# Vill-Lab/2023-TIFS-ISTVT

Hardware: AMD Instinct MI355X
Metric: clips/sec (BxTx3x224x224 fwd+bwd) (higher is better)
Workload: dtype bf16; 1 GPU; C2: B=32/GPU T=8 224x224 full ISTVT (Xception stem + 12-layer DSTTr) train step (fwd+bwd+grad all-reduce+SGD), random-init weights; global_batch=32, frames=8, size=224, depth=12, parallelism=dp1, early_allreduce=False, attn_fp8=False, dead_row_elimination=False, final_norm_class_rows_only=False, optimizer=SGD(momentum 0.9) fused, step_graphs=False

## Files before the change

### 2023-tifs-istvt_amd/csrc/attn_spatial.hip

```cpp
#include "common.h"
#include <type_traits>
#include <cstdlib>

constexpr int CHUNK = 128;
constexpr int NT = CHUNK / 16;
#ifdef ISTVT_SATTN_NOSTORE
#define SB_STORE4(p, v) do { if (scale < -1e30f) store4(p, v); } while (0)
#else
#define SB_STORE4(p, v) store4(p, v)
#endif
template <typename T, int DH> struct Pitch { static constexpr int v = DH + (sizeof(T) == 2 ? 16 : 8); };
#define LOG2E 1.4426950408889634f
#define LN2 0.6931471805599453f

template <typename T, int DH, int NTHR = 256>
__device__ __forceinline__ void stage_img(T* img, const T* __restrict__ src, long ld, int row0, int nrows, int tid) {
    constexpr int LDI = Pitch<T, DH>::v;
    constexpr int VPR = DH / 8;
    constexpr int NV = CHUNK * VPR / NTHR;
#pragma unroll
    for (int i = 0; i < NV; ++i) {
        const int v = tid + NTHR * i;
        const int row = v / VPR, col = (v % VPR) * 8;
        typename Mma<T>::frag f;
        if (row0 + row < nrows) f = frag_load(src + (long)(row0 + row) * ld + col);
        else f = Mma<T>::zero();
        if constexpr (sizeof(T) == 2) {
            *reinterpret_cast<bf16x8*>(img + row * LDI + col) = f;
        } else {
            float* p = (float*)(img + row * LDI + col);
            *reinterpret_cast<float4*>(p) = make_float4(f.v[0], f.v[1], f.v[2], f.v[3]);
            *reinterpret_cast<float4*>(p + 4) = make_float4(f.v[4], f.v[5], f.v[6], f.v[7]);
        }
    }
}

template <typename T, int DH, int NTHR>
struct StageRegs { typename Mma<T>::frag f[CHUNK * (DH / 8) / NTHR]; };
template <typename T, int DH, int NTHR>
__device__ __forceinline__ void stage_fetch(StageRegs<T, DH, NTHR>& rg, const T* __restrict__ src, long ld, int row0,
                                            int nrows, int tid) {
    constexpr int VPR = DH / 8;
    constexpr int NV = CHUNK * VPR / NTHR;
#pragma unroll
    for (int i = 0; i < NV; ++i) {
        const int v = tid + NTHR * i;
        const int row = v / VPR, col = (v % VPR) * 8;
        if (row0 + row < nrows) rg.f[i] = frag_load(src + (long)(row0 + row) * ld + col);
        else rg.f[i] = Mma<T>::zero();
    }
}
template <typename T, int DH, int NTHR>
__device__ __forceinline__ void stage_commit(T* img, const StageRegs<T, DH, NTHR>& rg, int tid, int rlim = CHUNK) {
    constexpr int LDI = Pitch<T, DH>::v;
    constexpr int VPR = DH / 8;
    constexpr int NV = CHUNK * VPR / NTHR;
#pragma unroll
    for (int i = 0; i < NV; ++i) {
        const int v = tid + NTHR * i;
        const int row = v / VPR, col = (v % VPR) * 8;
        if (row >= rlim) continue;
        if constexpr (sizeof(T) == 2) {
            *reinterpret_cast<bf16x8*>(img + row * LDI + col) = rg.f[i];
        } else {
            float* p = (float*)(img + row * LDI + col);
            *reinterpret_cast<float4*>(p) = make_float4(rg.f[i].v[0], rg.f[i].v[1], rg.f[i].v[2], rg.f[i].v[3]);
            *reinterpret_cast<float4*>(p + 4) = make_float4(rg.f[i].v[4], rg.f[i].v[5], rg.f[i].v[6], rg.f[i].v[7]);
        }
    }
}

template <typename T, int DH, int NTHR, int NCH>
__device__ __forceinline__ void stage_all2(T* imgA, const T* __restrict__ srcA, long ldA, T* imgB, const T* __restrict__ srcB,
                                           long ldB, int P, int tid, int img_rows) {
    constexpr int LDI = Pitch<T, DH>::v;
    StageRegs<T, DH, NTHR> ra[NCH], rb[NCH];
#pragma unroll
    for (int ch = 0; ch < NCH; ++ch) {
        if (ch * CHUNK < P) {
            stage_fetch(ra[ch], srcA, ldA, ch * CHUNK, P, tid);
            stage_fetch(rb[ch], srcB, ldB, ch * CHUNK, P, tid);
        }
    }
#pragma unroll
    for (int ch = 0; ch < NCH; ++ch) {
        if (ch * CHUNK < P) {
            stage_commit(imgA + ch * CHUNK * LDI, ra[ch], tid, img_rows - ch * CHUNK);
            stage_commit(imgB + ch * CHUNK * LDI, rb[ch], tid, img_rows - ch * CHUNK);
        }
    }
}

template <typename T>
__device__ __forceinline__ typename Mma<T>::frag row_frag(const T* __restrict__ src, long ld, int row, int nrows,
                                                           int col) {
    if (row < nrows) return frag_load(src + (long)row * ld + col);
    return Mma<T>::zero();
}

template <typename T>
__device__ __forceinline__ typename Mma<T>::frag acc_frag(const f32x4& lo, const f32x4& hi) {
    typename Mma<T>::frag f;
#pragma unroll
    for (int i = 0; i < 4; ++i) { Mma<T>::set(f, i, lo[i]); Mma<T>::set(f, 4 + i, hi[i]); }
    return f;
}

__device__ __forceinline__ long pack_fp8(const float (&v)[8]) {
    int lo = __builtin_amdgcn_cvt_pk_fp8_f32(v[0], v[1], 0, false);
    lo = __builtin_amdgcn_cvt_pk_fp8_f32(v[2], v[3], lo, true);
    int hi = __builtin_amdgcn_cvt_pk_fp8_f32(v[4], v[5], 0, false);
    hi = __builtin_amdgcn_cvt_pk_fp8_f32(v[6], v[7], hi, true);
    return (long)(((unsigned long)(unsigned)hi << 32) | (unsigned)lo);
}
__device__ __forceinline__ long to_fp8(const bf16x8& f) {
    float v[8];
#pragma unroll
    for (int i = 0; i < 8; ++i) v[i] = (float)f[i];
    return pack_fp8(v);
}
__device__ __forceinline__ long to_fp8(const f32frag& f) { return pack_fp8(f.v); }
__device__ __forceinline__ void mma8(f32x4& c, long a, long b) { c = __builtin_amdgcn_mfma_f32_16x16x32_fp8_fp8(a, b, c, 0, 0, 0); }
constexpr float P8_SCALE = 256.f;

__device__ __forceinline__ float group_max(float v) { return xgroup_max(v); }
__device__ __forceinline__ float group_sum(float v) { return xgroup_sum(v); }

#ifndef ISTVT_SATTN_RES_MAX
#define ISTVT_SATTN_RES_MAX 2
#endif
constexpr int RES_CHUNKS_MAX = ISTVT_SATTN_RES_MAX;
extern __shared__ __attribute__((aligned(16))) char sattn_dyn[];
__host__ __device__ inline int res_img_rows(int P) { return (P + 31) & ~31; }

template <typename T, int DH, int U, bool FP8 = false, int RES = 0>
__global__ __launch_bounds__(512 / U, (U == 1 && RES < 3) ? 4 : 1) void sattn_fwd_kernel(const T* __restrict__ qkv, T* __restrict__ out,
                                                        float* __restrict__ lse, int P, int heads, float scale, long ldqkv, long ldo) {
    constexpr int LDI = Pitch<T, DH>::v, KS = DH / 32, DT = DH / 16;
    __shared__ __attribute__((aligned(16))) T smem_st[RES ? 8 : 2 * CHUNK * LDI];
    const int img_rows = RES ? res_img_rows(P) : CHUNK;
    T* Kimg = RES ? reinterpret_cast<T*>(sattn_dyn) : smem_st;
    T* Vimg = Kimg + img_rows * LDI;
    const int tid = threadIdx.x, lane = tid & 63, wave = tid >> 6, g = lane >> 4, r = lane & 15;
    const int prob = blockIdx.y, h = prob % heads, bf = prob / heads;
    const int inner = heads * DH;
    const long ld = ldqkv;
    const T* base = qkv + (long)bf * P * ld;
#ifdef ISTVT_SATTN_DIAG
    const T* base_kv = qkv;
    const T* qp = (ISTVT_SATTN_DIAG >= 2 ? qkv : base + h * DH);
    const T* kp = base_kv + inner;
    const T* vp = base_kv + 2 * inner;
#else
    const T* qp = base + h * DH;
    const T* kp = base + inner + h * DH;
    const T* vp = base + 2 * inner + h * DH;
#endif
    const float c = scale * LOG2E;
    constexpr int NBLK = RES ? RES : 1;
    typename Mma<T>::frag qf_pre[NBLK][U][KS];
#pragma unroll
    for (int qi = 0; qi < NBLK; ++qi)
#pragma unroll
        for (int u = 0; u < U; ++u)
#pragma unroll
            for (int ks = 0; ks < KS; ++ks)
                qf_pre[qi][u][ks] = row_frag<T>(qp, ld, (RES ? qi : (int)blockIdx.x) * 128 + wave * 16 * U + 16 * u + r, P,
                                                32 * ks + 8 * g);
    if constexpr (RES) {
        stage_all2<T, DH, 512 / U, RES>(Kimg, kp, ld, Vimg, vp, ld, P, tid, img_rows);
        __syncthreads();
    }
#pragma unroll
  for (int qi = 0; qi < NBLK; ++qi) {
    const int qblk = RES ? qi : (int)blockIdx.x;
    const int q0 = qblk * 128 + wave * 16 * U;
    const bool active = q0 < P;
    if (RES && !active) break;

    typename Mma<T>::frag qf[U][KS];
    long q8[U][KS];
#pragma unroll
    for (int u = 0; u < U; ++u)
#pragma unroll
        for (int ks = 0; ks < KS; ++ks) {
            qf[u][ks] = qf_pre[qi][u][ks];
            if constexpr (FP8) q8[u][ks] = to_fp8(qf[u][ks]);
        }

    f32x4 o[DT][U];
    float m_run[U], l_run[U];
#pragma unroll
    for (int u = 0; u < U; ++u) {
        m_run[u] = -INFINITY; l_run[u] = 0.f;
#pragma unroll
        for (int dt = 0; dt < DT; ++dt) o[dt][u] = f32x4{0, 0, 0, 0};
    }

    auto chunk = [&](const int c0, auto tail_c) {
        constexpr bool TAIL = decltype(tail_c)::value;
        const T* const Kimg_c = RES ? Kimg + (c0 / CHUNK) * CHUNK * LDI : Kimg;
        const T* const Vimg_c = RES ? Vimg + (c0 / CHUNK) * CHUNK * LDI : Vimg;
        f32x4 s[NT][U];
#pragma unroll
        for (int t = 0; t < NT; ++t) {
#pragma unroll
            for (int u = 0; u < U; ++u) s[t][u] = f32x4{0, 0, 0, 0};
            if (!TAIL || c0 + 16 * t < P) {
#pragma unroll
                for (int ks = 0; ks < KS; ++ks) {
                    typename Mma<T>::frag kf = frag_load(Kimg_c + (16 * t + r) * LDI + 32 * ks + 8 * g);
                    if constexpr (FP8) {
                        const long k8 = to_fp8(kf);
#pragma unroll
                        for (int u = 0; u < U; ++u) mma8(s[t][u], k8, q8[u][ks]);
                    } else {
#pragma unroll
                        for (int u = 0; u < U; ++u) Mma<T>::mma(s[t][u], kf, qf[u][ks]);
                    }
                }
            }
        }
#pragma unroll
        for (int u = 0; u < U; ++u) {
            float mx = -INFINITY;
#pragma unroll
            for (int t = 0; t < NT; ++t) {
                if (TAIL && c0 + 16 * t >= P) continue;
                if (TAIL && c0 + 16 * t + 16 > P) {
#pragma unroll
                    for (int j = 0; j < 4; ++j) s[t][u][j] = (c0 + 16 * t + 4 * g + j < P) ? s[t][u][j] : -INFINITY;
                }
#pragma unroll
                for (int j = 0; j < 4; ++j) mx = fmaxf(mx, s[t][u][j]);
            }
            mx = group_max(mx) * c;
            const float m_new = fmaxf(m_run[u], mx);
            const float alpha = fast_exp2(m_run[u] - m_new);
            float sum = 0.f;
#pragma unroll
            for (int t = 0; t < NT; ++t) {
                if (TAIL && c0 + 16 * t >= P) continue;
#pragma unroll
                for (int j = 0; j < 4; ++j) {
                    const float pv = fast_exp2(fmaf(s[t][u][j], c, -m_new));
                    s[t][u][j] = pv;
                    sum += pv;
                }
            }
            sum = group_sum(sum);
            l_run[u] = l_run[u] * alpha + sum;
            m_run[u] = m_new;
#pragma unroll
            for (int dt = 0; dt < DT; ++dt) o[dt][u] *= alpha;
        }
#pragma unroll
        for (int ss = 0; ss < NT / 2; ++ss) {
            if (!TAIL || c0 + 32 * ss < P) {
                typename Mma<T>::frag pf[U];
                long p8[U];
#pragma unroll
                for (int u = 0; u < U; ++u) {
                    if constexpr (FP8) {
                        const f32x4 &lo = s[2 * ss][u], &hi = s[2 * ss + 1][u];
                        const float pv[8] = {lo[0] * P8_SCALE, lo[1] * P8_SCALE, lo[2] * P8_SCALE, lo[3] * P8_SCALE,
                                             hi[0] * P8_SCALE, hi[1] * P8_SCALE, hi[2] * P8_SCALE, hi[3] * P8_SCALE};
                        p8[u] = pack_fp8(pv);
                    } else {
                        pf[u] = acc_frag<T>(s[2 * ss][u], s[2 * ss + 1][u]);
                    }
                }
#pragma unroll
                for (int dt = 0; dt < DT; ++dt) {
                    typename Mma<T>::frag vf =
                        frag_load_tr(Vimg_c, LDI, 32 * ss + 4 * g, 32 * ss + 16 + 4 * g, 16 * dt, r);
                    if constexpr (FP8) {
                        const long v8 = to_fp8(vf);
#pragma unroll
                        for (int u = 0; u < U; ++u) mma8(o[dt][u], v8, p8[u]);
                    } else {
#pragma unroll
                        for (int u = 0; u < U; ++u) Mma<T>::mma(o[dt][u], vf, pf[u]);
                    }
                }
            }
        }
    };
    if constexpr (RES) {
        for (int c0 = 0; c0 < P; c0 += CHUNK) {
            if (c0 + CHUNK > P) chunk(c0, std::true_type{});
            else chunk(c0, std::false_type{});
        }
    } else {
        StageRegs<T, DH, 512 / U> kreg, vreg;
        stage_fetch(kreg, kp, ld, 0, P, tid);
        stage_fetch(vreg, vp, ld, 0, P, tid);
        for (int c0 = 0; c0 < P; c0 += CHUNK) {
            if (c0) __syncthreads();
            stage_commit(Kimg, kreg, tid);
            stage_commit(Vimg, vreg, tid);
            __syncthreads();
            if (c0 + CHUNK < P) {
                stage_fetch(kreg, kp, ld, c0 + CHUNK, P, tid);
                stage_fetch(vreg, vp, ld, c0 + CHUNK, P, tid);
            }
            if (!active) continue;
            if (c0 + CHUNK > P) chunk(c0, std::true_type{});
            else chunk(c0, std::false_type{});
        }
        if (!active) return;
    }
#pragma unroll
    for (int u = 0; u < U; ++u) {
        const int q = q0 + 16 * u + r;
        if (q >= P) continue;
        const float inv = 1.0f / l_run[u];
        const float oinv = FP8 ? inv * (1.0f / P8_SCALE) : inv;
        T* op = out + ((long)bf * P + q) * ldo + h * DH;
#pragma unroll
        for (int dt = 0; dt < DT; ++dt) {
            float v[4] = {o[dt][u][0] * oinv, o[dt][u][1] * oinv, o[dt][u][2] * oinv, o[dt][u][3] * oinv};
            store4(op + 16 * dt + 4 * g, v);
        }
        if (g == 0) {
            float2* st = reinterpret_cast<float2*>(lse) + ((long)bf * P + q) * heads + h;
            *st = make_float2(m_run[u], inv);
        }
    }
  }
}

template <typename T, int DH, int U, int NBLK> struct SattnKeep {
    typename Mma<T>::frag q[NBLK][U][DH / 32], d[NBLK][U][DH / 32];
};

template <typename T, int DH, int U, bool FP8 = false, int RES = 0, bool FUSED = false>
__device__ __forceinline__ void sattn_dq_body(const T* __restrict__ qkv, const T* __restrict__ out,
                                              const T* __restrict__ dout, const float* __restrict__ lse,
                                              float* __restrict__ delta, T* __restrict__ dqkv, int P,
                                              int heads, float scale, long ldqkv, long ldo,
                                              SattnKeep<T, DH, U, RES ? RES : 1>* keep = nullptr) {
    static_assert(!FUSED || RES, "the fused backward is the keys-resident form");
    constexpr int LDI = Pitch<T, DH>::v, KS = DH / 32, DT = DH / 16;
    __shared__ __attribute__((aligned(16))) T smem_st[RES ? 8 : 2 * CHUNK * LDI];
    const int img_rows = RES ? res_img_rows(P) : CHUNK;
    T* Kimg = RES ? reinterpret_cast<T*>(sattn_dyn) : smem_st;
    T* Vimg = Kimg + img_rows * LDI;
    const int tid = threadIdx.x, lane = tid & 63, wave = tid >> 6, g = lane >> 4, r = lane & 15;
    const int prob = blockIdx.y, h = prob % heads, bf = prob / heads;
    const int inner = heads * DH;
    const long ld = ldqkv;
    const T* base = qkv + (long)bf * P * ld;
    const T* qp = base + h * DH;
    const T* kp = base + inner + h * DH;
    const T* vp = base + 2 * inner + h * DH;
    const T* op = out + (long)bf * P * ldo + h * DH;
    const T* dop = dout + (long)bf * P * ldo + h * DH;
    const float c = scale * LOG2E;
    constexpr int NBLK = RES ? RES : 1;
    typename Mma<T>::frag qf_pre[NBLK][U][KS], dof_pre[NBLK][U][KS], of_pre[NBLK][U][KS];
    float2 st_pre[NBLK][U];
#pragma unroll
    for (int qi = 0; qi < NBLK; ++qi)
#pragma unroll
        for (int u = 0; u < U; ++u) {
            const int q = (RES ? qi : (int)blockIdx.x) * 128 + wave * 16 * U + 16 * u + r;
#pragma unroll
            for (int ks = 0; ks < KS; ++ks) {
                qf_pre[qi][u][ks] = row_frag<T>(qp, ld, q, P, 32 * ks + 8 * g);
                dof_pre[qi][u][ks] = row_frag<T>(dop, ldo, q, P, 32 * ks + 8 * g);
                of_pre[qi][u][ks] = row_frag<T>(op, ldo, q, P, 32 * ks + 8 * g);
                if constexpr (FUSED) { keep->q[qi][u][ks] = qf_pre[qi][u][ks]; keep->d[qi][u][ks] = dof_pre[qi][u][ks]; }
            }
            st_pre[qi][u] = q < P ? reinterpret_cast<const float2*>(lse)[((long)bf * P + q) * heads + h] : make_float2(0.f, 0.f);
        }
    if constexpr (RES) {
        stage_all2<T, DH, 512 / U, RES>(Kimg, kp, ld, Vimg, vp, ld, P, tid, img_rows);
        __syncthreads();
    }
#pragma unroll
  for (int qi = 0; qi < NBLK; ++qi) {
    const int qblk = RES ? qi : (int)blockIdx.x;
    const int q0 = qblk * 128 + wave * 16 * U;
    const bool active = q0 < P;
    if (RES && !active) break;

    typename Mma<T>::frag qf[U][KS], dof[U][KS];
    long q8[U][KS];
    float lq[U], li[U], dl[U];
#pragma unroll
    for (int u = 0; u < U; ++u) {
        const int q = q0 + 16 * u + r;
        float part = 0.f;
#pragma unroll
        for (int ks = 0; ks < KS; ++ks) {
            qf[u][ks] = qf_pre[qi][u][ks];
            if constexpr (FP8) q8[u][ks] = to_fp8(qf[u][ks]);
            dof[u][ks] = dof_pre[qi][u][ks];
#pragma unroll
            for (int i = 0; i < 8; ++i) part += Mma<T>::get(dof[u][ks], i) * Mma<T>::get(of_pre[qi][u][ks], i);
        }
        dl[u] = group_sum(part);
        const float2 st = st_pre[qi][u];
        lq[u] = st.x - __builtin_amdgcn_logf(st.y); li[u] = st.y;
        if constexpr (FUSED) {
            float* stat1 = reinterpret_cast<float*>(Kimg + 2 * img_rows * LDI) + img_rows;
            if (g == 0 && q < img_rows) stat1[q] = dl[u];
        } else {
            if (q < P && g == 0) delta[((long)bf * P + q) * heads + h] = dl[u];
        }
    }

    f32x4 dq[DT][U];
#pragma unroll
    for (int dt = 0; dt < DT; ++dt)
#pragma unroll
        for (int u = 0; u < U; ++u) dq[dt][u] = f32x4{0, 0, 0, 0};

    StageRegs<T, DH, 512 / U> kreg, vreg;
    if constexpr (!RES) {
        stage_fetch(kreg, kp, ld, 0, P, tid);
        stage_fetch(vreg, vp, ld, 0, P, tid);
    }
    for (int c0 = 0; c0 < P; c0 += CHUNK) {
        if constexpr (!RES) {
            if (c0) __syncthreads();
            stage_commit(Kimg, kreg, tid);
            stage_commit(Vimg, vreg, tid);
            __syncthreads();
            if (c0 + CHUNK < P) {
                stage_fetch(kreg, kp, ld, c0 + CHUNK, P, tid);
                stage_fetch(vreg, vp, ld, c0 + CHUNK, P, tid);
            }
            if (!active) continue;
        }
        const T* const Kimg_c = RES ? Kimg + (c0 / CHUNK) * CHUNK * LDI : Kimg;
        const T* const Vimg_c = RES ? Vimg + (c0 / CHUNK) * CHUNK * LDI : Vimg;
        const bool tail = c0 + CHUNK > P;
#pragma unroll
        for (int ss = 0; ss < NT / 2; ++ss) {
            if (c0 + 32 * ss >= P) continue;
            f32x4 s[2][U], dp[2][U];
#pragma unroll
            for (int tt = 0; tt < 2; ++tt) {
#pragma unroll
                for (int u = 0; u < U; ++u) { s[tt][u] = f32x4{0, 0, 0, 0}; dp[tt][u] = f32x4{0, 0, 0, 0}; }
                const int krow = 32 * ss + 16 * tt + r;
                const bool straddle = tail && c0 + 32 * ss + 16 * tt + 16 > P;
#pragma unroll
                for (int ks = 0; ks < KS; ++ks) {
                    typename Mma<T>::frag kf = frag_load(Kimg_c + krow * LDI + 32 * ks + 8 * g);
                    typename Mma<T>::frag vf = frag_load(Vimg_c + krow * LDI + 32 * ks + 8 * g);
#pragma unroll
                    for (int u = 0; u < U; ++u) {
                        if constexpr (FP8) mma8(s[tt][u], to_fp8(kf), q8[u][ks]);
                        else Mma<T>::mma(s[tt][u], kf, qf[u][ks]);
                        Mma<T>::mma(dp[tt][u], vf, dof[u][ks]);
                    }
                }
                auto softmax_bwd = [&](auto masked) {
#pragma unroll
                    for (int u = 0; u < U; ++u)
#pragma unroll
                        for (int j = 0; j < 4; ++j) {
                            float pv = fast_exp2(fmaf(s[tt][u][j], c, -lq[u]));
                            if (decltype(masked)::value && c0 + 32 * ss + 16 * tt + 4 * g + j >= P) pv = 0.f;
                            s[tt][u][j] = pv * (dp[tt][u][j] - dl[u]);
                        }
                };
                if (straddle) softmax_bwd(std::true_type{});
                else softmax_bwd(std::false_type{});
            }
            typename Mma<T>::frag dsf[U];
#pragma unroll
            for (int u = 0; u < U; ++u) dsf[u] = acc_frag<T>(s[0][u], s[1][u]);
#pragma unroll
            for (int dt = 0; dt < DT; ++dt) {
                typename Mma<T>::frag kt = frag_load_tr(Kimg_c, LDI, 32 * ss + 4 * g, 32 * ss + 16 + 4 * g, 16 * dt, r);
#pragma unroll
                for (int u = 0; u < U; ++u) Mma<T>::mma(dq[dt][u], kt, dsf[u]);
            }
        }
    }
    if (!active) return;
#pragma unroll
    for (int u = 0; u < U; ++u) {
        const int q = q0 + 16 * u + r;
        if (q >= P) continue;
        T* dqp = dqkv + ((long)bf * P + q) * ld + h * DH;
#pragma unroll
        for (int dt = 0; dt < DT; ++dt) {
            float v[4] = {dq[dt][u][0] * scale, dq[dt][u][1] * scale, dq[dt][u][2] * scale, dq[dt][u][3] * scale};
            SB_STORE4(dqp + 16 * dt + 4 * g, v);
        }
    }
  }
}

template <typename T, int DH, int U, bool FP8 = false, int RES = 0>
__global__ __launch_bounds__(512 / U) void sattn_bwd_dq_kernel(const T* __restrict__ qkv, const T* __restrict__ out,
                                                           const T* __restrict__ dout, const float* __restrict__ lse,
                                                           float* __restrict__ delta, T* __restrict__ dqkv, int P,
                                                           int heads, float scale, long ldqkv, long ldo) {
    sattn_dq_body<T, DH, U, FP8, RES, false>(qkv, out, dout, lse, delta, dqkv, P, heads, scale, ldqkv, ldo);
}

template <typename T, int DH, int U, bool FP8 = false, int RES = 0, bool FUSED = false>
__device__ __forceinline__ void sattn_dkv_body(const T* __restrict__ qkv, const T* __restrict__ dout,
                                               const float* __restrict__ lse,
                                               const float* __restrict__ delta, T* __restrict__ dqkv,
                                               int P, int heads, float scale, long ldqkv, long ldo,
                                               const SattnKeep<T, DH, U, RES ? RES : 1>* keep = nullptr) {
    constexpr int LDI = Pitch<T, DH>::v, KS = DH / 32, DT = DH / 16;
    __shared__ __attribute__((aligned(16))) T smem_st[RES ? 8 : 2 * CHUNK * LDI];
    __shared__ __attribute__((aligned(16))) float stat_st[RES ? 4 : 2 * CHUNK];
    const int img_rows = RES ? res_img_rows(P) : CHUNK;
    T* Qimg = RES ? reinterpret_cast<T*>(sattn_dyn) : smem_st;
    T* Dimg = Qimg + img_rows * LDI;
    float* stat0 = RES ? reinterpret_cast<float*>(Dimg + img_rows * LDI) : stat_st;
    float* stat1 = stat0 + img_rows;
    const int tid = threadIdx.x, lane = tid & 63, wave = tid >> 6, g = lane >> 4, r = lane & 15;
    const int prob = blockIdx.y, h = prob % heads, bf = prob / heads;
    const int inner = heads * DH;
    const long ld = ldqkv;
    const T* base = qkv + (long)bf * P * ld;
    const T* qp = base + h * DH;
    const T* kp = base + inner + h * DH;
    const T* vp = base + 2 * inner + h * DH;
    const T* dop = dout + (long)bf * P * ldo + h * DH;
    const float c = scale * LOG2E;
    constexpr int NBLK = RES ? RES : 1;
    typename Mma<T>::frag kf_pre[NBLK][U][KS], vf_pre[NBLK][U][KS];
#pragma unroll
    for (int ki = 0; ki < NBLK; ++ki)
#pragma unroll
        for (int kt = 0; kt < U; ++kt)
#pragma unroll
            for (int ks = 0; ks < KS; ++ks) {
                const int key = (RES ? ki : (int)blockIdx.x) * 128 + wave * 16 * U + 16 * kt + r;
                if constexpr (FUSED) {
                    const int kr = min(key, img_rows - 1);
                    typename Mma<T>::frag kk = frag_load(Qimg + kr * LDI + 32 * ks + 8 * g);
                    typename Mma<T>::frag vv = frag_load(Dimg + kr * LDI + 32 * ks + 8 * g);
                    if (key >= P) {
#pragma unroll
                        for (int i = 0; i < 8; ++i) { Mma<T>::set(kk, i, 0.f); Mma<T>::set(vv, i, 0.f); }
                    }
                    kf_pre[ki][kt][ks] = kk;
                    vf_pre[ki][kt][ks] = vv;
                } else {
                    kf_pre[ki][kt][ks] = row_frag<T>(kp, ld, key, P, 32 * ks + 8 * g);
                    vf_pre[ki][kt][ks] = row_frag<T>(vp, ld, key, P, 32 * ks + 8 * g);
                }
            }
    if constexpr (FUSED) __syncthreads();
    if constexpr (RES) {
        if constexpr (FUSED) {
#pragma unroll
            for (int qi = 0; qi < NBLK; ++qi)
#pragma unroll
                for (int u = 0; u < U; ++u) {
                    const int row = qi * 128 + wave * 16 * U + 16 * u + r;
                    if (row < img_rows) {
#pragma unroll
                        for (int ks = 0; ks < KS; ++ks) {
                            *reinterpret_cast<typename Mma<T>::frag*>(Qimg + row * LDI + 32 * ks + 8 * g) = keep->q[qi][u][ks];
                            *reinterpret_cast<typename Mma<T>::frag*>(Dimg + row * LDI + 32 * ks + 8 * g) = keep->d[qi][u][ks];
                        }
                    }
                }
        } else {
            stage_all2<T, DH, 512 / U, RES>(Qimg, qp, ld, Dimg, dop, ldo, P, tid, img_rows);
        }
        for (int q = tid; q < img_rows; q += 512 / U) {
            const float2 st = q < P ? reinterpret_cast<const float2*>(lse)[((long)bf * P + q) * heads + h] : make_float2(0.f, 0.f);
            stat0[q] = st.x - __builtin_amdgcn_logf(st.y);
            if constexpr (FUSED) { if (q >= P) stat1[q] = 0.f; }
            else stat1[q] = q < P ? delta[((long)bf * P + q) * heads + h] : 0.f;
        }
        __syncthreads();
    }
#pragma unroll
  for (int ki = 0; ki < NBLK; ++ki) {
    const int kblk = RES ? ki : (int)blockIdx.x;
    const int k0 = kblk * 128 + wave * 16 * U;
    const bool active = k0 < P;
    if (RES && !active) break;

    typename Mma<T>::frag kf[U][KS], vf[U][KS];
    long k8[U][KS];
#pragma unroll
    for (int kt = 0; kt < U; ++kt)
#pragma unroll
        for (int ks = 0; ks < KS; ++ks) {
            kf[kt][ks] = kf_pre[ki][kt][ks];
            if constexpr (FP8) k8[kt][ks] = to_fp8(kf[kt][ks]);
            vf[kt][ks] = vf_pre[ki][kt][ks];
        }
    f32x4 dk[DT][U], dv[DT][U];
#pragma unroll
    for (int dt = 0; dt < DT; ++dt)
#pragma unroll
        for (int kt = 0; kt < U; ++kt) { dk[dt][kt] = f32x4{0, 0, 0, 0}; dv[dt][kt] = f32x4{0, 0, 0, 0}; }

    StageRegs<T, DH, 512 / U> qreg, dreg;
    float2 streg = make_float2(0.f, 0.f);
    float dlreg = 0.f;
    auto fetch = [&](int c0) {
        stage_fetch(qreg, qp, ld, c0, P, tid);
        stage_fetch(dreg, dop, ldo, c0, P, tid);
        if (tid < CHUNK) {
            const int q = c0 + tid;
            streg = q < P ? reinterpret_cast<const float2*>(lse)[((long)bf * P + q) * heads + h]
                          : make_float2(0.f, 0.f);
            dlreg = q < P ? delta[((long)bf * P + q) * heads + h] : 0.f;
        }
    };
    if constexpr (!RES) fetch(0);
    for (int c0 = 0; c0 < P; c0 += CHUNK) {
        if constexpr (!RES) {
            if (c0) __syncthreads();
            stage_commit(Qimg, qreg, tid);
            stage_commit(Dimg, dreg, tid);
            if (tid < CHUNK) {
                stat0[tid] = streg.x - __builtin_amdgcn_logf(streg.y);
                stat1[tid] = dlreg;
            }
            __syncthreads();
            if (c0 + CHUNK < P) fetch(c0 + CHUNK);
            if (!active) continue;
        }
        const T* const Qimg_c = RES ? Qimg + (c0 / CHUNK) * CHUNK * LDI : Qimg;
        const T* const Dimg_c = RES ? Dimg + (c0 / CHUNK) * CHUNK * LDI : Dimg;
        const float* const st0 = RES ? stat0 + c0 : stat0;
        const float* const st1 = RES ? stat1 + c0 : stat1;
#pragma unroll
        for (int ss = 0; ss < NT / 2; ++ss) {
            if (c0 + 32 * ss >= P) continue;
            f32x4 s[2][U], dp[2][U];
#pragma unroll
            for (int tt = 0; tt < 2; ++tt) {
#pragma unroll
                for (int kt = 0; kt < U; ++kt) { s[tt][kt] = f32x4{0, 0, 0, 0}; dp[tt][kt] = f32x4{0, 0, 0, 0}; }
                const int qrow = 32 * ss + 16 * tt + r;
#pragma unroll
                for (int ks = 0; ks < KS; ++ks) {
                    typename Mma<T>::frag qa = frag_load(Qimg_c + qrow * LDI + 32 * ks + 8 * g);
                    typename Mma<T>::frag da = frag_load(Dimg_c + qrow * LDI + 32 * ks + 8 * g);
#pragma unroll
                    for (int kt = 0; kt < U; ++kt) {
                        if constexpr (FP8) mma8(s[tt][kt], to_fp8(qa), k8[kt][ks]);
                        else Mma<T>::mma(s[tt][kt], qa, kf[kt][ks]);
                        Mma<T>::mma(dp[tt][kt], da, vf[kt][ks]);
                    }
                }
                const int qb = 32 * ss + 16 * tt + 4 * g;
                const float4 l4 = *reinterpret_cast<const float4*>(st0 + qb);
                const float4 d4 = *reinterpret_cast<const float4*>(st1 + qb);
                const float lv[4] = {l4.x, l4.y, l4.z, l4.w}, dv4[4] = {d4.x, d4.y, d4.z, d4.w};
#pragma unroll
                for (int kt = 0; kt < U; ++kt)
#pragma unroll
                    for (int j = 0; j < 4; ++j) {
                        const float pv = fast_exp2(fmaf(s[tt][kt][j], c, -lv[j]));
                        s[tt][kt][j] = pv;
                        dp[tt][kt][j] = pv * (dp[tt][kt][j] - dv4[j]);
                    }
            }
            typename Mma<T>::frag pf[U], dsf[U];
#pragma unroll
            for (int kt = 0; kt < U; ++kt) { pf[kt] = acc_frag<T>(s[0][kt], s[1][kt]); dsf[kt] = acc_frag<T>(dp[0][kt], dp[1][kt]); }
#pragma unroll
            for (int dt = 0; dt < DT; ++dt) {
                typename Mma<T>::frag dot_ = frag_load_tr(Dimg_c, LDI, 32 * ss + 4 * g, 32 * ss + 16 + 4 * g, 16 * dt, r);
                typename Mma<T>::frag qt_ = frag_load_tr(Qimg_c, LDI, 32 * ss + 4 * g, 32 * ss + 16 + 4 * g, 16 * dt, r);
#pragma unroll
                for (int kt = 0; kt < U; ++kt) {
                    Mma<T>::mma(dv[dt][kt], dot_, pf[kt]);
                    Mma<T>::mma(dk[dt][kt], qt_, dsf[kt]);
                }
            }
        }
    }
    if (!active) return;
#pragma unroll
    for (int kt = 0; kt < U; ++kt) {
        const int key = k0 + 16 * kt + r;
        if (key >= P) continue;
        T* dkp = dqkv + ((long)bf * P + key) * ld + inner + h * DH;
        T* dvp = dqkv + ((long)bf * P + key) * ld + 2 * inner + h * DH;
#pragma unroll
        for (int dt = 0; dt < DT; ++dt) {
            float a[4] = {dk[dt][kt][0] * scale, dk[dt][kt][1] * scale, dk[dt][kt][2] * scale, dk[dt][kt][3] * scale};
            float b[4] = {dv[dt][kt][0], dv[dt][kt][1], dv[dt][kt][2], dv[dt][kt][3]};
            SB_STORE4(dkp + 16 * dt + 4 * g, a);
            SB_STORE4(dvp + 16 * dt + 4 * g, b);
        }
    }
  }
}

template <typename T, int DH, int U, bool FP8 = false, int RES = 0>
__global__ __launch_bounds__(512 / U) void sattn_bwd_dkv_kernel(const T* __restrict__ qkv, const T* __restrict__ dout,
                                                            const float* __restrict__ lse,
                                                            const float* __restrict__ delta, T* __restrict__ dqkv,
                                                            int P, int heads, float scale, long ldqkv, long ldo) {
    sattn_dkv_body<T, DH, U, FP8, RES, false>(qkv, dout, lse, delta, dqkv, P, heads, scale, ldqkv, ldo);
}

template <typename T, int DH, bool FP8 = false, int NCH = 2>
__global__ __launch_bounds__(512) void sattn_bwd_fused_kernel(const T* __restrict__ qkv, const T* __restrict__ out,
                                                              const T* __restrict__ dout, const float* __restrict__ lse,
                                                              T* __restrict__ dqkv, int P, int heads, float scale,
                                                              long ldqkv, long ldo) {
    SattnKeep<T, DH, 1, NCH> keep;
    sattn_dq_body<T, DH, 1, FP8, NCH, true>(qkv, out, dout, lse, nullptr, dqkv, P, heads, scale, ldqkv, ldo, &keep);
    __syncthreads();
    sattn_dkv_body<T, DH, 1, FP8, NCH, true>(qkv, dout, lse, nullptr, dqkv, P, heads, scale, ldqkv, ldo, &keep);
}

#include "attn_spatial_pers.h"

#define DISPATCH_DH(DHV, ...)                                   \
    do {                                                        \
        if ((DHV) == 64) { constexpr int DH = 64; __VA_ARGS__; } \
        else if ((DHV) == 32) { constexpr int DH = 32; __VA_ARGS__; } \
        else return ISTVT_ERR_SHAPE;                            \
    } while (0)

template <typename K>
static int res_lds(K kernel, int P, int dh, bool with_stats, size_t* bytes) {
    const size_t b = 2ul * res_img_rows(P) * (dh + 16) * sizeof(bf16_t) + (with_stats ? 2ul * res_img_rows(P) * sizeof(float) : 0);
    *bytes = b;
    if (b > 65536 &&
        hipFuncSetAttribute(reinterpret_cast<const void*>(kernel), hipFuncAttributeMaxDynamicSharedMemorySize, (int)b) != hipSuccess)
        return ISTVT_ERR_LAUNCH;
    return ISTVT_OK;
}
#define DISPATCH_RC(PV, ...)                                     \
    do {                                                         \
        if ((PV) <= 2 * CHUNK) { constexpr int RC = 2; __VA_ARGS__; } \
        else { constexpr int RC = 3; __VA_ARGS__; }              \
    } while (0)
#define LAUNCH_RES(KERNEL, STATS, ...)                                                            \
    do {                                                                                          \
        size_t lds_ = 0;                                                                          \
        const int rc_ = res_lds(KERNEL, P, dh, STATS, &lds_);                                     \
        if (rc_) return rc_;                                                                      \
        hipLaunchKernelGGL(KERNEL, dim3(1, BF * heads), dim3(512), lds_, stream, __VA_ARGS__);    \
    } while (0)

extern "C" int istvt_attn_spatial_fwd(const void* qkv, long ldqkv, void* out, long ldo, float* lse, int BF, int P, int heads, int dh,
                                      float scale, int dtype, hipStream_t stream) {
    if (BF <= 0 || P <= 0 || heads <= 0) return ISTVT_ERR_SHAPE;
    if (ldqkv < 3L * heads * dh || ldo < (long)heads * dh || ldqkv % 8 || ldo % 8) return ISTVT_ERR_SHAPE;
    dim3 grid((P + 127) / 128, BF * heads);
    if (dtype == DT_BF16) {
        static const int pers = istvt_tune("ISTVT_SATTN_PERS", 1);
        if (pers && dh == 64 && P > CHUNK && P <= 240 && ldqkv * 2 * P < 0x7fffffffL) {
            const int cus = istvt_device_cus();
            const int nprob = BF * heads, ntt = (P - CHUNK + 15) / 16;
            const dim3 pgrid(nprob < cus ? nprob : cus);
#define SP_LAUNCH(NTTV)                                                                                                   \
            case NTTV: {                                                                                                  \
                static std::atomic<unsigned long long> lds_raised{0};                                                      \
                if (istvt_raise_lds_limit(lds_raised, reinterpret_cast<const void*>(sattn_fwd_pers_kernel<64, NTTV>),      \
                                          4 * spers::IMG_B) != ISTVT_OK)                                                   \
                    return ISTVT_ERR_LAUNCH;                                                                               \
                hipLaunchKernelGGL((sattn_fwd_pers_kernel<64, NTTV>), pgrid, dim3(1024), 4 * spers::IMG_B, stream,          \
                                   (const bf16_t*)qkv, (bf16_t*)out, lse, nprob, P, heads, scale, ldqkv, ldo);            \
            } break;
            switch (ntt) {
                SP_LAUNCH(1) SP_LAUNCH(2) SP_LAUNCH(3) SP_LAUNCH(4) SP_LAUNCH(5) SP_LAUNCH(6) SP_LAUNCH(7) SP_LAUNCH(8)
                default: return ISTVT_ERR_SHAPE;
            }
#undef SP_LAUNCH
            return istvt_check_launch();
        }
        if (P > CHUNK && P <= RES_CHUNKS_MAX * CHUNK) {
            DISPATCH_DH(dh, DISPATCH_RC(P, LAUNCH_RES((sattn_fwd_kernel<bf16_t, DH, 1, false, RC>), false, (const bf16_t*)qkv, (bf16_t*)out, lse,
                                       P, heads, scale, ldqkv, ldo)));
            return istvt_check_launch();
        }
        DISPATCH_DH(dh, hipLaunchKernelGGL((sattn_fwd_kernel<bf16_t, DH, 1>), grid, dim3(512), 0, stream,
                                           (const bf16_t*)qkv, (bf16_t*)out, lse, P, heads, scale, ldqkv, ldo));
        return istvt_check_launch();
    }
    dim3 block(256);
    DISPATCH_DTYPE(dtype, DISPATCH_DH(dh, hipLaunchKernelGGL((sattn_fwd_kernel<T, DH, 2>), grid, block, 0, stream,
                                                             (const T*)qkv, (T*)out, lse, P, heads, scale, ldqkv, ldo)));
    return istvt_check_launch();
}

extern "C" int istvt_attn_spatial_bwd(const void* qkv, long ldqkv, const void* out, const void* dout, long ldo, const float* lse,
                                      float* delta, void* dqkv, int BF, int P, int heads, int dh, float scale,
                                      int dtype, hipStream_t stream) {
    if (BF <= 0 || P <= 0 || heads <= 0) return ISTVT_ERR_SHAPE;
    if (ldqkv < 3L * heads * dh || ldo < (long)heads * dh || ldqkv % 8 || ldo % 8) return ISTVT_ERR_SHAPE;
    dim3 grid((P + 127) / 128, BF * heads);
    static const int fused = istvt_tune("ISTVT_SATTN_FUSED_BWD", 1);
    if (fused && dtype == DT_BF16 && P > CHUNK && P <= RES_CHUNKS_MAX * CHUNK) {
        DISPATCH_DH(dh, DISPATCH_RC(P, LAUNCH_RES((sattn_bwd_fused_kernel<bf16_t, DH, false, RC>), true, (const bf16_t*)qkv, (const bf16_t*)out,
                                   (const bf16_t*)dout, lse, (bf16_t*)dqkv, P, heads, scale, ldqkv, ldo)));
        return istvt_check_launch();
    }
    if (dtype == DT_BF16 && P > CHUNK && P <= RES_CHUNKS_MAX * CHUNK) {
        DISPATCH_DH(dh, DISPATCH_RC(P, {
            LAUNCH_RES((sattn_bwd_dq_kernel<bf16_t, DH, 1, false, RC>), false, (const bf16_t*)qkv, (const bf16_t*)out,
                       (const bf16_t*)dout, lse, delta, (bf16_t*)dqkv, P, heads, scale, ldqkv, ldo);
            LAUNCH_RES((sattn_bwd_dkv_kernel<bf16_t, DH, 1, false, RC>), true, (const bf16_t*)qkv, (const bf16_t*)dout, lse,
                       (const float*)delta, (bf16_t*)dqkv, P, heads, scale, ldqkv, ldo);
        }));
        return istvt_check_launch();
    }
    if (dtype == DT_BF16) {
        DISPATCH_DH(dh, {
            hipLaunchKernelGGL((sattn_bwd_dq_kernel<bf16_t, DH, 1>), grid, dim3(512), 0, stream, (const bf16_t*)qkv,
                               (const bf16_t*)out, (const bf16_t*)dout, lse, delta, (bf16_t*)dqkv, P, heads, scale, ldqkv, ldo);
            hipLaunchKernelGGL((sattn_bwd_dkv_kernel<bf16_t, DH, 1>), grid, dim3(512), 0, stream, (const bf16_t*)qkv,
                               (const bf16_t*)dout, lse, (const float*)delta, (bf16_t*)dqkv, P, heads, scale, ldqkv, ldo);
        });
        return istvt_check_launch();
    }
    dim3 block(256);
    DISPATCH_DTYPE(dtype, DISPATCH_DH(dh, {
        hipLaunchKernelGGL((sattn_bwd_dq_kernel<T, DH, 2>), grid, block, 0, stream, (const T*)qkv, (const T*)out,
                           (const T*)dout, lse, delta, (T*)dqkv, P, heads, scale, ldqkv, ldo);
        hipLaunchKernelGGL((sattn_bwd_dkv_kernel<T, DH, 2>), grid, block, 0, stream, (const T*)qkv, (const T*)dout, lse,
                           (const float*)delta, (T*)dqkv, P, heads, scale, ldqkv, ldo);
    }));
    return istvt_check_launch();
}

extern "C" int istvt_attn_spatial_fwd_fp8(const void* qkv, long ldqkv, void* out, long ldo, float* lse, int BF, int P, int heads, int dh,
                                          float scale, int dtype, hipStream_t stream) {
    if (BF <= 0 || P <= 0 || heads <= 0) return ISTVT_ERR_SHAPE;
    if (ldqkv < 3L * heads * dh || ldo < (long)heads * dh || ldqkv % 8 || ldo % 8) return ISTVT_ERR_SHAPE;
    if (dtype != DT_BF16) return ISTVT_ERR_DTYPE;
    dim3 grid((P + 127) / 128, BF * heads);
    if (P > CHUNK && P <= RES_CHUNKS_MAX * CHUNK) {
        DISPATCH_DH(dh, DISPATCH_RC(P, LAUNCH_RES((sattn_fwd_kernel<bf16_t, DH, 1, true, RC>), false, (const bf16_t*)qkv, (bf16_t*)out, lse, P,
                                   heads, scale, ldqkv, ldo)));
        return istvt_check_launch();
    }
    DISPATCH_DH(dh, hipLaunchKernelGGL((sattn_fwd_kernel<bf16_t, DH, 1, true>), grid, dim3(512), 0, stream,
                                       (const bf16_t*)qkv, (bf16_t*)out, lse, P, heads, scale, ldqkv, ldo));
    return istvt_check_launch();
}

extern "C" int istvt_attn_spatial_bwd_fp8(const void* qkv, long ldqkv, const void* out, const void* dout, long ldo, const float* lse,
                                          float* delta, void* dqkv, int BF, int P, int heads, int dh, float scale,
                                          int dtype, hipStream_t stream) {
    if (BF <= 0 || P <= 0 || heads <= 0) return ISTVT_ERR_SHAPE;
    if (ldqkv < 3L * heads * dh || ldo < (long)heads * dh || ldqkv % 8 || ldo % 8) return ISTVT_ERR_SHAPE;
    if (dtype != DT_BF16) return ISTVT_ERR_DTYPE;
    dim3 grid((P + 127) / 128, BF * heads);
    static const int fused = istvt_tune("ISTVT_SATTN_FUSED_BWD", 1);
    if (fused && P > CHUNK && P <= RES_CHUNKS_MAX * CHUNK) {
        DISPATCH_DH(dh, DISPATCH_RC(P, LAUNCH_RES((sattn_bwd_fused_kernel<bf16_t, DH, true, RC>), true, (const bf16_t*)qkv, (const bf16_t*)out,
                                   (const bf16_t*)dout, lse, (bf16_t*)dqkv, P, heads, scale, ldqkv, ldo)));
        return istvt_check_launch();
    }
    if (P > CHUNK && P <= RES_CHUNKS_MAX * CHUNK) {
        DISPATCH_DH(dh, DISPATCH_RC(P, {
            LAUNCH_RES((sattn_bwd_dq_kernel<bf16_t, DH, 1, true, RC>), false, (const bf16_t*)qkv, (const bf16_t*)out,
                       (const bf16_t*)dout, lse, delta, (bf16_t*)dqkv, P, heads, scale, ldqkv, ldo);
            LAUNCH_RES((sattn_bwd_dkv_kernel<bf16_t, DH, 1, true, RC>), true, (const bf16_t*)qkv, (const bf16_t*)dout, lse,
                       (const float*)delta, (bf16_t*)dqkv, P, heads, scale, ldqkv, ldo);
        }));
        return istvt_check_launch();
    }
    DISPATCH_DH(dh, {
        hipLaunchKernelGGL((sattn_bwd_dq_kernel<bf16_t, DH, 1, true>), grid, dim3(512), 0, stream, (const bf16_t*)qkv,
                           (const bf16_t*)out, (const bf16_t*)dout, lse, delta, (bf16_t*)dqkv, P, heads, scale, ldqkv, ldo);
        hipLaunchKernelGGL((sattn_bwd_dkv_kernel<bf16_t, DH, 1, true>), grid, dim3(512), 0, stream, (const bf16_t*)qkv,
                           (const bf16_t*)dout, lse, (const float*)delta, (bf16_t*)dqkv, P, heads, scale, ldqkv, ldo);
    });
    return istvt_check_launch();
}
```

Measured before the change: 647.3 clips/s.

## Add tail-specialised fused spatial attention backward kernel for 128<P<=256, dh=64

```diff
diff --git a/2023-tifs-istvt_amd/csrc/attn_spatial.hip b/2023-tifs-istvt_amd/csrc/attn_spatial.hip
--- a/2023-tifs-istvt_amd/csrc/attn_spatial.hip
+++ b/2023-tifs-istvt_amd/csrc/attn_spatial.hip
@@ -720,6 +720,7 @@
 }
 
 #include "attn_spatial_pers.h"
+#include "attn_spatial_bwd_spec.h"
 
 #define DISPATCH_DH(DHV, ...)                                   \
     do {                                                        \
@@ -792,6 +793,11 @@
     return istvt_check_launch();
 }
 
+static inline bool sattn_bwd_spec_wanted() {
+    const char* v = getenv("ISTVT_SATTN_BWD_SPEC");
+    return !(v && v[0] == '0' && v[1] == 0);
+}
+
 extern "C" int istvt_attn_spatial_bwd(const void* qkv, long ldqkv, const void* out, const void* dout, long ldo, const float* lse,
                                       float* delta, void* dqkv, int BF, int P, int heads, int dh, float scale,
                                       int dtype, hipStream_t stream) {
@@ -799,6 +805,26 @@
     if (ldqkv < 3L * heads * dh || ldo < (long)heads * dh || ldqkv % 8 || ldo % 8) return ISTVT_ERR_SHAPE;
     dim3 grid((P + 127) / 128, BF * heads);
     static const int fused = istvt_tune("ISTVT_SATTN_FUSED_BWD", 1);
+    if (fused && dtype == DT_BF16 && dh == 64 && P > CHUNK && P <= 2 * CHUNK && sattn_bwd_spec_wanted()) {
+        const int ntt = (P - CHUNK + 15) / 16;
+        const size_t lds = 2ul * res_img_rows(P) * (64 + 16) * sizeof(bf16_t) + 2ul * res_img_rows(P) * sizeof(float);
+#define SB_LAUNCH(NTTV)                                                                                                   \
+        case NTTV: {                                                                                                      \
+            static std::atomic<unsigned long long> lds_raised{0};                                                          \
+            if (lds > 65536 && istvt_raise_lds_limit(lds_raised, reinterpret_cast<const void*>(sattn_bwd_spec_kernel<NTTV>), \
+                                                     (int)lds) != ISTVT_OK)                                                \
+                return ISTVT_ERR_LAUNCH;                                                                                   \
+            hipLaunchKernelGGL((sattn_bwd_spec_kernel<NTTV>), dim3(1, BF * heads), dim3(512), lds, stream,                  \
+                               (const bf16_t*)qkv, (const bf16_t*)out, (const bf16_t*)dout, lse, (bf16_t*)dqkv, P, heads,   \
+                               scale, ldqkv, ldo);                                                                         \
+        } break;
+        switch (ntt) {
+            SB_LAUNCH(1) SB_LAUNCH(2) SB_LAUNCH(3) SB_LAUNCH(4) SB_LAUNCH(5) SB_LAUNCH(6) SB_LAUNCH(7) SB_LAUNCH(8)
+            default: return ISTVT_ERR_SHAPE;
+        }
+#undef SB_LAUNCH
+        return istvt_check_launch();
+    }
     if (fused && dtype == DT_BF16 && P > CHUNK && P <= RES_CHUNKS_MAX * CHUNK) {
         DISPATCH_DH(dh, DISPATCH_RC(P, LAUNCH_RES((sattn_bwd_fused_kernel<bf16_t, DH, false, RC>), true, (const bf16_t*)qkv, (const bf16_t*)out,
                                    (const bf16_t*)dout, lse, (bf16_t*)dqkv, P, heads, scale, ldqkv, ldo)));
diff --git a/2023-tifs-istvt_amd/csrc/attn_spatial_bwd_spec.h b/2023-tifs-istvt_amd/csrc/attn_spatial_bwd_spec.h
--- /dev/null
+++ b/2023-tifs-istvt_amd/csrc/attn_spatial_bwd_spec.h
@@ -0,0 +1,264 @@
+#pragma once
+
+namespace sbspec {
+enum { FULL = 0, STRADDLE = 1, ABSENT = 2 };
+
+template <int NTT> constexpr int tail_mode(int t) { return t < NTT - 1 ? FULL : t == NTT - 1 ? STRADDLE : ABSENT; }
+
+struct Lane {
+    const bf16_t *arow, *brow;
+    const bf16_t *atr, *btr;
+    const float *s0, *s1;
+};
+__device__ __forceinline__ bf16x8 tr_load(const bf16_t* lo, const bf16_t* hi) {
+    typedef short4v __attribute__((address_space(3))) * lds_ptr;
+    typedef short short8v __attribute__((ext_vector_type(8)));
+    const short4v a = __builtin_amdgcn_ds_read_tr16_b64_v4i16((lds_ptr)(lo));
+    const short4v b = __builtin_amdgcn_ds_read_tr16_b64_v4i16((lds_ptr)(hi));
+    short8v v;
+    v[0] = a[0]; v[1] = a[1]; v[2] = a[2]; v[3] = a[3]; v[4] = b[0]; v[5] = b[1]; v[6] = b[2]; v[7] = b[3];
+    return __builtin_bit_cast(bf16x8, v);
+}
+
+template <int ROW0, int M0, int M1>
+__device__ __forceinline__ void dq_pair(const Lane& L, const bf16x8 (&qf)[2], const bf16x8 (&dof)[2], const float c,
+                                        const float lq, const float dl, const int P, const int g, f32x4 (&dq)[4]) {
+    constexpr int LDI = Pitch<bf16_t, 64>::v;
+    f32x4 s[2];
+#pragma unroll
+    for (int tt = 0; tt < 2; ++tt) {
+        const int mode = tt ? M1 : M0;
+        s[tt] = f32x4{0, 0, 0, 0};
+        if (mode == ABSENT) continue;
+        f32x4 dp = f32x4{0, 0, 0, 0};
+#pragma unroll
+        for (int ks = 0; ks < 2; ++ks) {
+            const bf16x8 kf = frag_load(L.arow + (ROW0 + 16 * tt) * LDI + 32 * ks);
+            const bf16x8 vf = frag_load(L.brow + (ROW0 + 16 * tt) * LDI + 32 * ks);
+            Mma<bf16_t>::mma(s[tt], kf, qf[ks]);
+            Mma<bf16_t>::mma(dp, vf, dof[ks]);
+        }
+#pragma unroll
+        for (int j = 0; j < 4; ++j) {
+            float pv = fast_exp2(fmaf(s[tt][j], c, -lq));
+            if (mode == STRADDLE && ROW0 + 16 * tt + 4 * g + j >= P) pv = 0.f;
+            s[tt][j] = pv * (dp[j] - dl);
+        }
+    }
+    const bf16x8 dsf = acc_frag<bf16_t>(s[0], s[1]);
+#pragma unroll
+    for (int dt = 0; dt < 4; ++dt) {
+        const bf16x8 kt = tr_load(L.atr + ROW0 * LDI + 16 * dt, L.atr + (ROW0 + 16) * LDI + 16 * dt);
+        Mma<bf16_t>::mma(dq[dt], kt, dsf);
+    }
+}
+
+template <int ROW0, int M1>
+__device__ __forceinline__ void dkv_pair(const Lane& L, const bf16x8 (&kf)[2], const bf16x8 (&vf)[2], const float c,
+                                         f32x4 (&dk)[4], f32x4 (&dv)[4]) {
+    constexpr int LDI = Pitch<bf16_t, 64>::v;
+    f32x4 s[2], dp[2];
+#pragma unroll
+    for (int tt = 0; tt < 2; ++tt) {
+        s[tt] = f32x4{0, 0, 0, 0};
+        dp[tt] = f32x4{0, 0, 0, 0};
+        if (tt && M1 == ABSENT) continue;
+#pragma unroll
+        for (int ks = 0; ks < 2; ++ks) {
+            const bf16x8 qa = frag_load(L.arow + (ROW0 + 16 * tt) * LDI + 32 * ks);
+            const bf16x8 da = frag_load(L.brow + (ROW0 + 16 * tt) * LDI + 32 * ks);
+            Mma<bf16_t>::mma(s[tt], qa, kf[ks]);
+            Mma<bf16_t>::mma(dp[tt], da, vf[ks]);
+        }
+        const float4 l4 = *reinterpret_cast<const float4*>(L.s0 + ROW0 + 16 * tt);
+        const float4 d4 = *reinterpret_cast<const float4*>(L.s1 + ROW0 + 16 * tt);
+        const float lv[4] = {l4.x, l4.y, l4.z, l4.w}, dv4[4] = {d4.x, d4.y, d4.z, d4.w};
+#pragma unroll
+        for (int j = 0; j < 4; ++j) {
+            const float pv = fast_exp2(fmaf(s[tt][j], c, -lv[j]));
+            s[tt][j] = pv;
+            dp[tt][j] = pv * (dp[tt][j] - dv4[j]);
+        }
+    }
+    const bf16x8 pf = acc_frag<bf16_t>(s[0], s[1]), dsf = acc_frag<bf16_t>(dp[0], dp[1]);
+#pragma unroll
+    for (int dt = 0; dt < 4; ++dt) {
+        const bf16x8 dot_ = tr_load(L.btr + ROW0 * LDI + 16 * dt, L.btr + (ROW0 + 16) * LDI + 16 * dt);
+        const bf16x8 qt_ = tr_load(L.atr + ROW0 * LDI + 16 * dt, L.atr + (ROW0 + 16) * LDI + 16 * dt);
+        Mma<bf16_t>::mma(dv[dt], dot_, pf);
+        Mma<bf16_t>::mma(dk[dt], qt_, dsf);
+    }
+}
+
+template <int PAIR0, int PAIR1, typename F>
+__device__ __forceinline__ void for_pairs(F&& f) {
+    if constexpr (PAIR0 < PAIR1) {
+        f(std::integral_constant<int, PAIR0>{});
+        for_pairs<PAIR0 + 1, PAIR1>(f);
+    }
+}
+}
+
+template <int NTT>
+__global__ __launch_bounds__(512, 4) void sattn_bwd_spec_kernel(const bf16_t* __restrict__ qkv, const bf16_t* __restrict__ out,
+                                                             const bf16_t* __restrict__ dout, const float* __restrict__ lse,
+                                                             bf16_t* __restrict__ dqkv, int P, int heads, float scale,
+                                                             long ldqkv, long ldo) {
+    using namespace sbspec;
+    static_assert(NTT >= 1 && NTT <= 8, "128 < P <= 256");
+    constexpr int DH = 64, LDI = Pitch<bf16_t, DH>::v, KS = DH / 32, DT = DH / 16;
+    constexpr int NPT = (NTT + 1) / 2;
+    constexpr int IMG_ROWS = CHUNK + 32 * NPT;
+    bf16_t* Aimg = reinterpret_cast<bf16_t*>(sattn_dyn);
+    bf16_t* Bimg = Aimg + IMG_ROWS * LDI;
+    float* stat0 = reinterpret_cast<float*>(Bimg + IMG_ROWS * LDI);
+    float* stat1 = stat0 + IMG_ROWS;
+    constexpr int LAST0 = CHUNK + 32 * (NPT - 1);
+    const int tid = threadIdx.x, lane = tid & 63, g = lane >> 4, r = lane & 15;
+    const int wave = __builtin_amdgcn_readfirstlane(tid >> 6);
+    const int prob = blockIdx.y, h = prob % heads, bf = prob / heads;
+    const int inner = heads * DH;
+    const long ld = ldqkv;
+    const bf16_t* base = qkv + (long)bf * P * ld;
+    const bf16_t* qp = base + h * DH;
+    const bf16_t* kp = base + inner + h * DH;
+    const bf16_t* vp = base + 2 * inner + h * DH;
+    const bf16_t* op = out + (long)bf * P * ldo + h * DH;
+    const bf16_t* dop = dout + (long)bf * P * ldo + h * DH;
+    const float c = scale * LOG2E;
+    const Lane L = {Aimg + r * LDI + 8 * g, Bimg + r * LDI + 8 * g, Aimg + (4 * g + (r >> 2)) * LDI + 4 * (r & 3),
+                    Bimg + (4 * g + (r >> 2)) * LDI + 4 * (r & 3), stat0 + 4 * g, stat1 + 4 * g};
+    const bool live1 = wave < NTT, full1 = wave < NTT - 1;
+
+    bf16x8 qf[2][KS], dof[2][KS], of[2][KS];
+    float2 st[2];
+    auto rows_load = [&](const int qi, auto masked) {
+        const int q = qi * CHUNK + wave * 16 + r;
+        const bool ok = !decltype(masked)::value || q < P;
+#pragma unroll
+        for (int ks = 0; ks < KS; ++ks) {
+            const int col = 32 * ks + 8 * g;
+            qf[qi][ks] = ok ? frag_load(qp + (long)q * ld + col) : Mma<bf16_t>::zero();
+            dof[qi][ks] = ok ? frag_load(dop + (long)q * ldo + col) : Mma<bf16_t>::zero();
+            of[qi][ks] = ok ? frag_load(op + (long)q * ldo + col) : Mma<bf16_t>::zero();
+        }
+        st[qi] = ok ? reinterpret_cast<const float2*>(lse)[((long)bf * P + q) * heads + h] : make_float2(0.f, 0.f);
+    };
+    rows_load(0, std::false_type{});
+    if (full1) rows_load(1, std::false_type{});
+    else if (live1) rows_load(1, std::true_type{});
+    else {
+#pragma unroll
+        for (int ks = 0; ks < KS; ++ks) qf[1][ks] = dof[1][ks] = Mma<bf16_t>::zero();
+    }
+
+    {
+        constexpr int VPR = DH / 8, NV = CHUNK * VPR / 512;
+        bf16x8 kr[2][NV], vr[2][NV];
+#pragma unroll
+        for (int ch = 0; ch < 2; ++ch)
+#pragma unroll
+            for (int i = 0; i < NV; ++i) {
+                const int v = tid + 512 * i, row = ch * CHUNK + v / VPR, col = (v % VPR) * 8;
+                constexpr int RPI = 512 / VPR;
+                if (ch * CHUNK + RPI * i >= IMG_ROWS) continue;
+                const bool sure = ch == 0 || RPI * (i + 1) <= 16 * (NTT - 1);
+                const bool ok = sure || row < P;
+                kr[ch][i] = ok ? frag_load(kp + (long)row * ld + col) : Mma<bf16_t>::zero();
+                vr[ch][i] = ok ? frag_load(vp + (long)row * ld + col) : Mma<bf16_t>::zero();
+            }
+#pragma unroll
+        for (int ch = 0; ch < 2; ++ch)
+#pragma unroll
+            for (int i = 0; i < NV; ++i) {
+                const int v = tid + 512 * i, row = ch * CHUNK + v / VPR, col = (v % VPR) * 8;
+                constexpr int RPI = 512 / VPR;
+                if (ch * CHUNK + RPI * i >= IMG_ROWS) continue;
+                if (ch * CHUNK + RPI * (i + 1) > IMG_ROWS && row >= IMG_ROWS) continue;
+                *reinterpret_cast<bf16x8*>(Aimg + row * LDI + col) = kr[ch][i];
+                *reinterpret_cast<bf16x8*>(Bimg + row * LDI + col) = vr[ch][i];
+            }
+    }
+    __syncthreads();
+
+    float lq[2], dl[2];
+#pragma unroll
+    for (int qi = 0; qi < 2; ++qi) {
+        if (qi && !live1) break;
+        const int q = qi * CHUNK + wave * 16 + r;
+        float part = 0.f;
+#pragma unroll
+        for (int ks = 0; ks < KS; ++ks)
+#pragma unroll
+            for (int i = 0; i < 8; ++i) part += (float)dof[qi][ks][i] * (float)of[qi][ks][i];
+        dl[qi] = group_sum(part);
+        lq[qi] = st[qi].x - __builtin_amdgcn_logf(st[qi].y);
+        if (g == 0) { stat0[q] = lq[qi]; stat1[q] = dl[qi]; }
+    }
+    auto dq_block = [&](const int qi) {
+        const int q = qi * CHUNK + wave * 16 + r;
+        f32x4 dq[DT];
+#pragma unroll
+        for (int dt = 0; dt < DT; ++dt) dq[dt] = f32x4{0, 0, 0, 0};
+        for_pairs<0, NT / 2 + NPT - 1>([&](auto pair) {
+            dq_pair<32 * decltype(pair)::value, FULL, FULL>(L, qf[qi], dof[qi], c, lq[qi], dl[qi], P, g, dq);
+        });
+        dq_pair<LAST0, tail_mode<NTT>(2 * NPT - 2), tail_mode<NTT>(2 * NPT - 1)>(L, qf[qi], dof[qi], c, lq[qi], dl[qi], P, g, dq);
+        if (qi && q >= P) return;
+        bf16_t* dqp = dqkv + ((long)bf * P + q) * ld + h * DH;
+#pragma unroll
+        for (int dt = 0; dt < DT; ++dt) {
+            float v[4] = {dq[dt][0] * scale, dq[dt][1] * scale, dq[dt][2] * scale, dq[dt][3] * scale};
+            SB_STORE4(dqp + 16 * dt + 4 * g, v);
+        }
+    };
+    dq_block(0);
+    if (live1) dq_block(1);
+
+    bf16x8 kf[2][KS], vf[2][KS];
+#pragma unroll
+    for (int ki = 0; ki < 2; ++ki) {
+        if (ki && !live1) break;
+        const int key = ki * CHUNK + wave * 16 + r;
+#pragma unroll
+        for (int ks = 0; ks < KS; ++ks) {
+            kf[ki][ks] = frag_load(Aimg + key * LDI + 32 * ks + 8 * g);
+            vf[ki][ks] = frag_load(Bimg + key * LDI + 32 * ks + 8 * g);
+        }
+    }
+    __syncthreads();
+#pragma unroll
+    for (int qi = 0; qi < 2; ++qi) {
+        if (qi && wave >= 2 * NPT) break;
+        const int row = qi * CHUNK + wave * 16 + r;
+#pragma unroll
+        for (int ks = 0; ks < KS; ++ks) {
+            *reinterpret_cast<bf16x8*>(Aimg + row * LDI + 32 * ks + 8 * g) = qf[qi][ks];
+            *reinterpret_cast<bf16x8*>(Bimg + row * LDI + 32 * ks + 8 * g) = dof[qi][ks];
+        }
+    }
+    __syncthreads();
+
+    auto dkv_block = [&](const int ki) {
+        f32x4 dk[DT], dv[DT];
+#pragma unroll
+        for (int dt = 0; dt < DT; ++dt) { dk[dt] = f32x4{0, 0, 0, 0}; dv[dt] = f32x4{0, 0, 0, 0}; }
+        for_pairs<0, NT / 2 + NPT - 1>([&](auto pair) {
+            dkv_pair<32 * decltype(pair)::value, FULL>(L, kf[ki], vf[ki], c, dk, dv);
+        });
+        dkv_pair<LAST0, tail_mode<NTT>(2 * NPT - 1)>(L, kf[ki], vf[ki], c, dk, dv);
+        const int key = ki * CHUNK + wave * 16 + r;
+        if (ki && key >= P) return;
+        bf16_t* dkp = dqkv + ((long)bf * P + key) * ld + inner + h * DH;
+        bf16_t* dvp = dqkv + ((long)bf * P + key) * ld + 2 * inner + h * DH;
+#pragma unroll
+        for (int dt = 0; dt < DT; ++dt) {
+            float a[4] = {dk[dt][0] * scale, dk[dt][1] * scale, dk[dt][2] * scale, dk[dt][3] * scale};
+            float b[4] = {dv[dt][0], dv[dt][1], dv[dt][2], dv[dt][3]};
+            SB_STORE4(dkp + 16 * dt + 4 * g, a);
+            SB_STORE4(dvp + 16 * dt + 4 * g, b);
+        }
+    };
+    dkv_block(0);
+    if (live1) dkv_block(1);
+}
```

After: 650.2 clips/s, median of 6. About the same (+0.5%).
